# drscotthawley/flocoder

Measured on NVIDIA B200. Metric: samples/sec, 50-step RK4 latent sampling, higher is better.
Workload: dtype bf16

## Files before the change

### flocoder_b200/csrc/api.cu

```cuda
#include <cuda_fp16.h>
#include <math.h>
#include <stdarg.h>
#include <stdio.h>
#include <stdlib.h>
#include <string.h>

#include <algorithm>
#include <map>
#include <memory>
#include <string>
#include <vector>

#include "flo_internal.h"

namespace flo {

int conv_umma_smem_bytes(const ConvUmmaParams& p);

static thread_local std::string g_last_error;
void set_error(const char* fmt, ...) {
    char buf[1024];
    va_list ap;
    va_start(ap, fmt);
    vsnprintf(buf, sizeof(buf), fmt, ap);
// ... 1334 lines not shown
        }
    }
    for (size_t i = 0; i < h.bufs.size(); ++i) {
        const Buf& bf = h.bufs[i];
        snprintf(line, sizeof(line), "buf %3zu %-34s C=%d %dx%d %s bytes_ps=%zu live=[%d,%d] off_ps=%zu\n", i, bf.name.c_str(), bf.C, bf.H,
                 bf.W, bf.bf16 ? "bf16" : "f32 ", bf.bytes_ps, bf.def, bf.last, bf.off_ps);
        t += line;
    }
    if (h.spec.fused) {
        FusedBuilder fb(h, h.ftensors, h.fstages, 4);
        rc = fb.build();
        if (rc) return rc;
        snprintf(line, sizeof(line), "fused: %d stages, %d boundary tensors, %zu bytes/sample\n", (int)h.fstages.size(),
                 (int)h.ftensors.size(), h.farena_ps);
        t += line;
        for (size_t i = 0; i < h.fstages.size(); ++i) {
            const FStage& st = h.fstages[i];
            if (st.kind == 0) {
                const ChainParams& c = st.cp;
                snprintf(line, sizeof(line), "stage %2zu chain %-12s %dx%d nb=%d mt=%d strips=%d steps=%d loads=%d smem=%d (slots %d, ring %dx%d) tmem=%d nsplit=%d ctas=%d\n",
                         i, st.name.c_str(), c.H, c.W, c.nb, c.n_mtiles, c.strips, c.n_steps, c.n_loads, c.smem_bytes, c.ring_off,
                         c.n_ring, c.ring_slot_bytes, c.tmem_cols, c.nsplit, c.nsplit * ((B + c.nb - 1) / c.nb));
                t += line;
                for (int k = 0; k < c.n_steps; ++k) {
                    const ChainStep& cs = c.st[k];
                    snprintf(line, sizeof(line), "      step %d: conv=%d k=%d cin=%d+%d n=%d chunks=%dx%d res=%d(%dx%d) epi=%d C=%d G=%d film=%d resmode=%d out_slot=%d out_g=%d un=%d up=%d pn=%d final=%d a0=%d a1=%d\n",
                             k, cs.has_conv, cs.ksize, cs.a0_ncb * 8, cs.a1_ncb * 8, cs.n, cs.slices, cs.slices_per_chunk, cs.has_res,
                             cs.res_slices, cs.res_slices_per_chunk, cs.epi, cs.C, cs.groups, cs.film_off, cs.res_mode, cs.out_slot_off,
                             cs.out_g, cs.out_un_g, cs.out_up_g, cs.pn_g, cs.final, cs.a0_off, cs.a1_off);
                    t += line;
                }
            } else {
                const AttnFusedParams& a = st.ap;
                snprintf(line, sizeof(line), "stage %2zu attn  %-12s %dx%d C=%d nb=%d n=%d n_pad=%d mt=%d full=%d smem=%d plane=%d tmem=%d cols(k=%d v=%d ctx=%d q=%d out=%d proj=%d) ctas=%d\n",
                         i, st.name.c_str(), a.H, a.W, a.C, a.nb, a.n, a.n_pad, a.n_mtiles, a.full, a.smem_bytes, a.plane_bytes, a.tmem_cols,
                         a.col_k, a.col_v, a.col_ctx, a.col_q, a.col_out, a.col_proj, (B + a.nb - 1) / a.nb);
                t += line;
            }
        }
        for (size_t i = 0; i < h.ftensors.size(); ++i) {
            snprintf(line, sizeof(line), "ftensor %2zu %-24s C=%d %dx%d off_ps=%zu\n", i, h.ftensors[i].name.c_str(), h.ftensors[i].C,
                     h.ftensors[i].H, h.ftensors[i].W, h.ftensors[i].off_ps);
            t += line;
        }
    }
    if (out && cap > 0) snprintf(out, cap, "%s", t.c_str());
    return (int)t.size();
}

static void op_cost(const Handle& h, const Op& op, double& fl, double& by) {
    const Spec& s = h.spec;
    const double ob = s.bf16 ? 2.0 : 4.0;
    fl = 0; by = 0;
    const double hw = (double)op.H * op.W;
    switch (op.kind) {
        case OP_INIT:
            fl = 2.0 * hw * s.dim * s.channels;
            by = hw * (s.channels * 4.0 + s.dim * (ob + (s.bf16 ? 4.0 : 0.0)));
            break;
        case OP_CONV: {
            const double cin = (op.ncb0 + op.ncb1) * 8.0;
            fl = 2.0 * hw * op.cout * cin * op.ksize * op.ksize;
            by = hw * cin * ob + hw * op.cout * ((op.out_m >= 0 ? 4.0 : 0.0) + (op.out_o >= 0 ? ob : 0.0) + (op.res >= 0 ? 4.0 : 0.0));
        } break;
        case OP_GN:
            by = hw * op.C * (4.0 + (op.res >= 0 ? 4.0 : 0.0) + (op.out_m >= 0 ? 4.0 : 0.0) + (op.out_o >= 0 ? ob : 0.0) +
                              (op.out_un >= 0 ? ob : 0.0) + (op.out_up >= 0 ? 4.0 * ob : 0.0));
            fl = 10.0 * hw * op.C;
            break;
// ... 194 lines not shown
```

### flocoder_b200/csrc/flo_internal.h

```cpp
#pragma once
#include <cuda_runtime.h>
#include <cuda_bf16.h>
#include <cuda.h>
#include <stdint.h>
#include <string>
#include <vector>

#include "../../include/flocoder_b200.h"

namespace flo {

enum StageKind : int {
    ST_PLAIN = 0,
    ST_RK1 = 1,
    ST_RK2 = 2,
    ST_RK3 = 3,
    ST_RK4 = 4,
    ST_EULER = 5,
    ST_CFG_COND = 6
};
enum StageFlags : int {
    SF_CFG_COMBINE = 1,
    SF_CFG_2B = 2
};
// ... 204 lines not shown
    int ones_off;
    int fast;
    int max_c;
    int g_max, coef_n, cpar_n;
    int wide;
    int ring_off, ring_slot_bytes, n_ring, n_ring_deep;
    int stats_off, bar_off, smem_bytes, tmem_cols;
    int tab_off, tab_n;
    int wtab_off, n_chunks;
    int tabs_off;
    int nsplit;
    int xpart_off;
    int fmt;
    int film_dim;
    int cin0, dim, channels;
    int init_w_off, init_b_off, final_w_off, final_b_off;
    const uint16_t* wblob;
    const float* fblob;
    void* gt[CH_MAX_GT];
    Ctrl* ctrl;
    long long* dbg;
};

struct AttnFusedParams {
    int epi_warps;
    int B, H, W, C, nb, n, n_pad, n_mtiles;
    int full;
    int ktrans;
    int small;
    int fmt;
    unsigned wq_off, wk_off, wv_off, wo_off;
    int qkv_chunks, qkv_S, o_chunks, o_S;
    int bo_off, gamma_off, beta_off;
    int xh_off, p_off, v_off, ct_off, kmax_off, stats_off;
    int plane_bytes;
    int ring_off, ring_slot_bytes, n_ring, bar_off, smem_bytes, tmem_cols;
    int zero_off, zero_bytes;
    int col_k, col_v, col_ctx, col_q, col_out, col_proj;
    const uint16_t* wblob;
    const float* fblob;
    const void* x2;
    void* out; void* out_un; void* out_up;
    long long* dbg;
};

cudaError_t fused_configure();
int fused_max_active_clusters(int nsplit, int smem_bytes);
cudaError_t launch_chain(const ChainParams& p, const CUtensorMap* maps, int grid, cudaStream_t s);
cudaError_t launch_attn_fused(const AttnFusedParams& p, const CUtensorMap& xh_map, int grid, cudaStream_t s);


}
```

### flocoder_b200/csrc/fused_attn.cu

```cuda
#include "flo_internal.h"
#include "fused_common.cuh"

namespace flo {

struct RingA { int cc; };
__device__ __forceinline__ uint64_t desc64(uint32_t lo, uint32_t hi) {
    uint64_t d;
    asm("mov.b64 %0, {%1, %2};" : "=l"(d) : "r"(lo), "r"(hi));
    return d;
}
constexpr int ATTN_RING = 4;

__device__ __forceinline__ void attn_issue_chunk(const AttnFusedParams& p, uint32_t smem_base, uint32_t bar_full, uint32_t bar_empty,
                                                 int g, int qkv_bytes, int o_bytes) {
    const int qc = p.qkv_chunks;
    const uint16_t* w; int ci, bytes;
    if (g < qc) { w = p.wblob + p.wk_off; ci = g; bytes = qkv_bytes; }
    else if (g < 2 * qc) { w = p.wblob + p.wv_off; ci = g - qc; bytes = qkv_bytes; }
    else if (g < 3 * qc) { w = p.wblob + p.wq_off; ci = g - 2 * qc; bytes = qkv_bytes; }
    else { w = p.wblob + p.wo_off; ci = g - 3 * qc; bytes = o_bytes; }
    const int slot = g & (ATTN_RING - 1);
    if (g >= ATTN_RING) mbar_wait(bar_empty + 8 * slot, ((g / ATTN_RING) - 1) & 1);
    mbar_expect_tx(bar_full + 8 * slot, (uint32_t)bytes);
    bulk_load_1d(smem_base + p.ring_off + slot * p.ring_slot_bytes, reinterpret_cast<const uint8_t*>(w) + (size_t)ci * bytes,
// ... 86 lines not shown
}

template <int M>
__device__ __forceinline__ void colmax_halve(float (&v)[16], bool upper, int o) {
#pragma unroll
    for (int j = 0; j < M / 2; ++j) {
        const float send = upper ? v[j] : v[j + M / 2];
        const float keep = upper ? v[j + M / 2] : v[j];
        v[j] = fmaxf(keep, __shfl_xor_sync(0xffffffffu, send, o));
    }
}
template <int SEG>
__device__ __forceinline__ int colmax16(float (&v)[16], int lane) {
    int chan = 0;
    if (SEG == 32) {
        colmax_halve<16>(v, lane & 16, 16); chan += (lane & 16) ? 8 : 0;
        colmax_halve<8>(v, lane & 8, 8);    chan += (lane & 8) ? 4 : 0;
        colmax_halve<4>(v, lane & 4, 4);    chan += (lane & 4) ? 2 : 0;
        colmax_halve<2>(v, lane & 2, 2);    chan += (lane & 2) ? 1 : 0;
        v[0] = fmaxf(v[0], __shfl_xor_sync(0xffffffffu, v[0], 1));
    } else if (SEG == 16) {
        colmax_halve<16>(v, lane & 8, 8); chan += (lane & 8) ? 8 : 0;
        colmax_halve<8>(v, lane & 4, 4);  chan += (lane & 4) ? 4 : 0;
        colmax_halve<4>(v, lane & 2, 2);  chan += (lane & 2) ? 2 : 0;
        colmax_halve<2>(v, lane & 1, 1);  chan += (lane & 1) ? 1 : 0;
    } else {
        colmax_halve<16>(v, lane & 2, 2); chan += (lane & 2) ? 8 : 0;
        colmax_halve<8>(v, lane & 1, 1);  chan += (lane & 1) ? 4 : 0;
    }
    return chan;
}

template <int NT = 0, int FMTK = -1>
__global__ void __launch_bounds__(ATTN_MAX_THREADS) k_attn(const __grid_constant__ CUtensorMap tm_xh,
                                                        const __grid_constant__ AttnFusedParams p) {
    extern __shared__ __align__(128) uint8_t smem[];
    constexpr bool LEAN = NT > 0;
    const int fmt_k = FMTK >= 0 ? FMTK : p.fmt;
    const bool is_full = LEAN ? false : (p.full != 0);
    const bool is_kt = LEAN;
    const int warp = threadIdx.x >> 5, lane = threadIdx.x & 31, tid = threadIdx.x;
    const int EW = NT == 2 ? 16 : (NT == 1 ? 8 : p.epi_warps), n_epi = EW * 32, n_thr = (int)blockDim.x;
    const int n_mtiles_k = NT ? NT : p.n_mtiles;
    const bool n_ge32 = LEAN ? true : (p.n >= 32);
    const int w_prod = EW, w_mma = EW + 1;
    const uint32_t smem_base = smem_u32(smem);
    const uint32_t bar_full = smem_base + p.bar_off;
    const uint32_t bar_empty = bar_full + 8 * MAX_WSTAGES;
    const uint32_t bar_load = bar_empty + 8 * MAX_WSTAGES;
    const uint32_t bar_mma = bar_load + 8;
    const uint32_t bar_epi = bar_mma + 8;
    const uint32_t tmem_slot = bar_epi + 8;
    volatile uint32_t* tmem_slot_ptr = reinterpret_cast<volatile uint32_t*>(smem + p.bar_off + 16 * MAX_WSTAGES + 24);
    constexpr int NCH = 128;
    const int b0 = (int)blockIdx.x * p.nb;
    if (p.dbg && tid == 0 && blockIdx.x == 0) p.dbg[100] = global_ns();
    const int n = p.n, n_pad = p.n_pad, C = p.C;
    const uint32_t plane = (uint32_t)p.plane_bytes;
    const uint32_t xh_plane = (uint32_t)(p.nb * n) * 16u;
    const int lgn = 31 - __clz(n);
    const int mtS = (n + 127) >> 7;

    if (warp == w_prod && lane == 0) {
        for (int i = 0; i < p.n_ring; ++i) { mbar_init(bar_full + 8 * i, 1); mbar_init(bar_empty + 8 * i, 1); }
        mbar_init(bar_load, 1);
        mbar_init(bar_mma, 1);
        mbar_init(bar_epi, n_epi);
        asm volatile("fence.mbarrier_init.release.cluster;" ::: "memory");
    }
    if (warp == w_mma) tmem_alloc(tmem_slot, (uint32_t)p.tmem_cols);
    const bool all_live = !is_full && p.n_pad == p.n && ((p.nb * p.n) & 127) == 0 && b0 + p.nb <= p.B;
    if (!all_live)
        for (int i = tid * 16; i < p.zero_bytes; i += n_thr * 16)
            *reinterpret_cast<uint4*>(smem + p.zero_off + i) = make_uint4(0, 0, 0, 0);
    fence_proxy_async();
    tc_fence_before();
    __syncthreads();
    tc_fence_after();
    const uint32_t tmem_base = *tmem_slot_ptr;
    long long* dbg = (blockIdx.x == 0) ? p.dbg : nullptr;
    if (dbg && tid == 0) dbg[64] = clock64();
    if (dbg && tid == 0) dbg[101] = global_ns();
    const int qkv_bytes = p.qkv_S * 128 * 32, o_bytes = p.o_S * C * 32;

    if (warp == w_prod) {
        if (lane == 0) {
            const int total = 3 * p.qkv_chunks + p.o_chunks, pre = min(ATTN_RING, total);
            for (int g = 0; g < pre; ++g) attn_issue_chunk(p, smem_base, bar_full, bar_empty, g, qkv_bytes, o_bytes);
            griddep_wait();
            mbar_expect_tx(bar_load, (uint32_t)(C >> 3) * xh_plane);
            tma_load_5d(smem_base + p.xh_off, &tm_xh, bar_load, 0, 0, 0, b0, 0);
            for (int g = pre; g < total; ++g) attn_issue_chunk(p, smem_base, bar_full, bar_empty, g, qkv_bytes, o_bytes);
        }
    } else if (warp == w_mma) {
        {
            RingA rs{0};
            mbar_wait(bar_load, 0);
            tc_fence_after();
            if (dbg && lane == 0) dbg[0] = clock64();
            const bool tr = is_kt != 0;
            auto conv_T = [&](int col) {
                const uint32_t idesc = make_idesc16(128, p.nb * n, fmt_k, 0, 0);
                for (int ci = 0; ci < p.qkv_chunks; ++ci) {
                    const int slot = rs.cc & (ATTN_RING - 1);
                    mbar_wait(bar_full + 8 * slot, (rs.cc / ATTN_RING) & 1);
                    tc_fence_after();
                    if (elect_one()) {
                        for (int sl = 0; sl < p.qkv_S; ++sl) {
                            const uint32_t a_addr = smem_base + p.ring_off + (uint32_t)slot * (uint32_t)p.ring_slot_bytes + (uint32_t)sl * 4096u;
                            const uint32_t b_addr = smem_base + p.xh_off + (uint32_t)(ci * p.qkv_S + sl) * 2u * xh_plane;
                            umma_bf16(tmem_base + (uint32_t)col, make_smem_desc(a_addr, 2048u, 128u), make_smem_desc(b_addr, xh_plane, 128u), idesc,
                                      (ci * p.qkv_S + sl) > 0 ? 1u : 0u);
                        }
                        umma_commit(bar_empty + 8 * slot);
                    }
                    __syncwarp();
                    ++rs.cc;
                }
            };
            if (tr) {
// ... 2 lines not shown
            } else {
            attn_conv(p, smem_base, tmem_base, bar_full, bar_empty, rs, p.xh_off, xh_plane, NCH, 128, p.col_k, p.qkv_chunks, p.qkv_S);
            attn_conv(p, smem_base, tmem_base, bar_full, bar_empty, rs, p.xh_off, xh_plane, NCH, 128, p.col_v, p.qkv_chunks, p.qkv_S);
            }
            if (is_full) attn_conv(p, smem_base, tmem_base, bar_full, bar_empty, rs, p.xh_off, xh_plane, NCH, 128, p.col_q, p.qkv_chunks, p.qkv_S);
            if (dbg && lane == 0) dbg[1] = clock64();
            if (elect_one()) umma_commit(bar_mma);
            __syncwarp();
            int ph = 0;
            if (!is_full) {
                named_bar_sync(2, n_epi + 32); ++ph;
                tc_fence_after();
                if (dbg && lane == 0) dbg[8] = clock64();
                const uint32_t idesc_ctx = make_idesc16(128, NCH + 16, fmt_k, 1, 1);
                {
                    const int nb = p.nb, col_ctx = p.col_ctx;
                    const uint32_t p_off = p.p_off, v_off = p.v_off;
                    if (tr) {
                        const uint32_t idesc_t = make_idesc16(128, NCH + 16, fmt_k, 0, 0);
                        if (elect_one())
                            for (int s = 0; s < nb; ++s)
                                for (int ks = 0; ks < n / 16; ++ks) {
                                    const uint32_t pl = (uint32_t)(s * (n >> 3) + 2 * ks);
                                    umma_bf16(tmem_base + (uint32_t)(col_ctx + s * (NCH + 16)), make_smem_desc(smem_base + p_off + pl * 2048u, 2048u, 128u),
                                              make_smem_desc(smem_base + v_off + pl * 2304u, 2304u, 128u), idesc_t, ks > 0 ? 1u : 0u);
                                }
                    } else if (elect_one())
                        for (int s = 0; s < nb; ++s)
                            for (int ks = 0; ks < n_pad / 16; ++ks) {
                                const uint32_t roff = (uint32_t)(s * n_pad + ks * 16) * 16u;
                                umma_bf16(tmem_base + (uint32_t)(col_ctx + s * (NCH + 16)), make_smem_desc(smem_base + p_off + roff, 128u, plane),
                                          make_smem_desc(smem_base + v_off + roff, 128u, plane), idesc_ctx, ks > 0 ? 1u : 0u);
                            }
                    __syncwarp();
                }
                attn_conv(p, smem_base, tmem_base, bar_full, bar_empty, rs, p.xh_off, xh_plane, NCH, 128, p.col_q, p.qkv_chunks, p.qkv_S);
                if (dbg && lane == 0) dbg[9] = clock64();
                if (elect_one()) umma_commit(bar_mma);
                __syncwarp();
                named_bar_sync(2, n_epi + 32); ++ph;
                tc_fence_after();
                if (dbg && lane == 0) dbg[16] = clock64();
                const uint32_t idesc_out = make_idesc16(128, 32, fmt_k, 0, 0);
                {
                    const int nb = p.nb, col_out = p.col_out;
                    const uint32_t p_off = p.p_off, ct_off = p.ct_off;
                    if (elect_one()) {
                        for (int s = 0; s < nb; ++s)
                            for (int t = 0; t < mtS; ++t)
                                for (int h = 0; h < 4; ++h)
                                    for (int k = 0; k < 2; ++k) {
                                        const uint32_t a_addr = smem_base + p_off + (uint32_t)(4 * h + 2 * k) * plane +
                                                                (uint32_t)(s * n_pad + t * 128) * 16u;
                                        const uint32_t b_addr = smem_base + ct_off + (uint32_t)(s * 4 + h) * 2048u + (uint32_t)k * 1024u;
                                        umma_bf16(tmem_base + (uint32_t)(col_out + (s * mtS + t) * NCH + h * 32),
                                                  make_smem_desc(a_addr, plane, 128u), make_smem_desc(b_addr, 512u, 128u), idesc_out,
                                                  k > 0 ? 1u : 0u);
                                    }
                        umma_commit(bar_mma);
                    }
                    __syncwarp();
                }
            }
            named_bar_sync(2, n_epi + 32); ++ph;
            tc_fence_after();
            if (dbg && lane == 0) dbg[24] = clock64();
            attn_conv(p, smem_base, tmem_base, bar_full, bar_empty, rs, is_full ? p.p_off : p.v_off, plane, C, C, p.col_proj,
                      p.o_chunks, p.o_S);
            if (elect_one()) umma_commit(bar_mma);
            __syncwarp();
        }
    } else {
        const int quad = warp & 3, grp = warp >> 2;
        const int r = quad * 32 + lane;
        const int et = grp * 128 + r;
        const int half = EW == 16 ? (grp & 1) : 0;
        const int t0 = half, tstep = EW == 16 ? 2 : 1;
        const int cpart = EW == 16 ? (grp >> 1) : (EW == 8 ? grp : 0), ncp = EW >= 8 ? 2 : 1;
        const int ch_lo = cpart * (NCH / ncp), ch_hi = ch_lo + NCH / ncp;
        const uint32_t tlane = tmem_base + ((uint32_t)(quad * 32) << 16);
        auto esync = [&]() { named_bar_sync(1, n_epi); };
        float* kmax = reinterpret_cast<float*>(smem + p.kmax_off);
        float* kpart = kmax + p.nb * 128;
        float2* rowstat = reinterpret_cast<float2*>(smem + p.stats_off);
        float2* partial = rowstat + n_mtiles_k * 128;
        float2* stat = partial + 256;
        int ph = 0;
        float* par = reinterpret_cast<float*>(stat + 128);
        for (int c = et; c < C; c += n_epi) {
            par[c] = p.fblob[p.bo_off + c];
            par[128 + c] = is_full ? 1.0f : p.fblob[p.gamma_off + c];
            par[256 + c] = is_full ? 0.0f : p.fblob[p.beta_off + c];
        }
        esync();
        griddep_wait();
        mbar_wait(bar_load, 0);
        mbar_wait(bar_mma, ph & 1); ++ph;
        tc_fence_after();
        if (dbg && r == 0) dbg[2] = clock64();
        if (!is_full) {
          if (is_kt) {
            const int d = r;
            const int col0 = grp * 64, s = col0 >> lgn, gps = n >> 6;
            float mx = -INFINITY;
#pragma unroll
            for (int c = 0; c < 64; c += 32) {
                uint32_t ua[16], ub[16];
                tmem_ld16_issue(tlane + (uint32_t)(p.col_k + col0 + c), ua);
                tmem_ld16_issue(tlane + (uint32_t)(p.col_k + col0 + c + 16), ub);
                tmem_ld_wait();
                float m4[4] = {mx, -INFINITY, -INFINITY, -INFINITY};
#pragma unroll
                for (int j = 0; j < 16; ++j) { m4[j & 3] = fmaxf(m4[j & 3], __uint_as_float(ua[j])); m4[j & 3] = fmaxf(m4[j & 3], __uint_as_float(ub[j])); }
                mx = fmaxf(fmaxf(m4[0], m4[1]), fmaxf(m4[2], m4[3]));
            }
            kpart[grp * 128 + d] = mx;
            for (int pl = et; pl < (p.nb * n) >> 3; pl += n_epi) {
                const float ones[8] = {1.f, 1.f, 1.f, 1.f, 1.f, 1.f, 1.f, 1.f};
                *reinterpret_cast<uint4*>(smem + p.v_off + (uint32_t)pl * 2304u + 128u * 16u) = pack8(ones, fmt_k);
            }
            if (dbg && r == 0) dbg[3] = clock64();
            esync();
            for (int g = 0; g < gps; ++g) mx = fmaxf(mx, kpart[(s * gps + g) * 128 + d]);
#pragma unroll 2
            for (int c = 0; c < 64; c += 16) {
                uint32_t ku[16], vu[16];
// ... 84 lines not shown
                for (int c16 = ch_lo; c16 < ch_hi; c16 += 16) {
                    uint32_t ku[16], vu[16];
                    tmem_ld16_issue(tlane + (uint32_t)(p.col_k + t * NCH + c16), ku);
                    tmem_ld16_issue(tlane + (uint32_t)(p.col_v + t * NCH + c16), vu);
                    tmem_ld_wait();
                    if (!valid) continue;
                    float kv[16], vv[16];
#pragma unroll
                    for (int j = 0; j < 16; ++j) { kv[j] = __uint_as_float(ku[j]); vv[j] = __uint_as_float(vu[j]); }
                    const float4* km4 = reinterpret_cast<const float4*>(kmax + s * 128 + c16);
#pragma unroll
                    for (int k4 = 0; k4 < 4; ++k4) {
                        const float4 m4 = km4[k4];
                        kv[4 * k4] = fast_exp(kv[4 * k4] - m4.x); kv[4 * k4 + 1] = fast_exp(kv[4 * k4 + 1] - m4.y);
                        kv[4 * k4 + 2] = fast_exp(kv[4 * k4 + 2] - m4.z); kv[4 * k4 + 3] = fast_exp(kv[4 * k4 + 3] - m4.w);
                    }
                    uint8_t* pd = smem + p.p_off + (uint32_t)(c16 >> 3) * plane + row_off;
                    uint8_t* vd = smem + p.v_off + (uint32_t)(c16 >> 3) * plane + row_off;
                    *reinterpret_cast<uint4*>(pd) = pack8(kv, fmt_k);
                    *reinterpret_cast<uint4*>(pd + plane) = pack8(kv + 8, fmt_k);
                    *reinterpret_cast<uint4*>(vd) = pack8(vv, fmt_k);
                    *reinterpret_cast<uint4*>(vd + plane) = pack8(vv + 8, fmt_k);
                }
                if (valid && cpart == 0) {
                    const float ones[8] = {1.f, 1.f, 1.f, 1.f, 1.f, 1.f, 1.f, 1.f};
                    *reinterpret_cast<uint4*>(smem + p.v_off + (uint32_t)(NCH >> 3) * plane + row_off) = pack8(ones, fmt_k);
                }
            }
            if (dbg && r == 0) dbg[4] = clock64();
            fence_proxy_async();
            tc_fence_before();
            named_bar_arrive(2, n_epi + 32);
          }
            mbar_wait(bar_mma, ph & 1); ++ph;
            tc_fence_after();
            if (dbg && r == 0) dbg[10] = clock64();
            {
                const int h = quad, d = lane;
                for (int s = t0; s < p.nb; s += tstep) {
                    uint32_t u0[16], u1[16], us[16];
                    tmem_ld16_issue(tlane + (uint32_t)(p.col_ctx + s * (NCH + 16) + h * 32), u0);
                    tmem_ld16_issue(tlane + (uint32_t)(p.col_ctx + s * (NCH + 16) + h * 32 + 16), u1);
                    tmem_ld16_issue(tlane + (uint32_t)(p.col_ctx + s * (NCH + 16) + NCH), us);
                    tmem_ld_wait();
                    const int e_lo = cpart * (32 / ncp), e_hi = e_lo + 32 / ncp;
                    float c0[16], c1[16];
#pragma unroll
                    for (int j = 0; j < 16; ++j) { c0[j] = __uint_as_float(u0[j]); c1[j] = __uint_as_float(u1[j]); }
                    const float inv = 0.17677669529663687f * fast_rcp(__uint_as_float(us[0]));
                    uint8_t* base = smem + p.ct_off + (uint32_t)(s * 4 + h) * 2048u + (uint32_t)(d >> 3) * 512u + (uint32_t)(d & 7) * 2u;
#pragma unroll
                    for (int e = 0; e < 32; ++e) {
                        if (e < e_lo || e >= e_hi) continue;
                        const float val = (e < 16 ? c0[e] : c1[e - 16]) * inv;
                        const uint32_t u = pack2(val, 0.f, fmt_k);
                        *reinterpret_cast<uint16_t*>(base + (uint32_t)(e >> 3) * 128u + (uint32_t)(e & 7) * 16u) = (uint16_t)(u & 0xFFFFu);
                    }
                }
            }
            for (int t = t0; t < n_mtiles_k; t += tstep) {
                const int rd = t * 128 + r, s = rd >> lgn, px = rd & (n - 1);
                const bool valid = s < p.nb && b0 + s < p.B;
                const uint32_t row_off = (uint32_t)(s * n_pad + px) * 16u;
                for (int h2 = cpart * (4 / ncp); h2 < (cpart + 1) * (4 / ncp); h2 += 2) {
                    uint32_t qu[2][32];
#pragma unroll
                    for (int k = 0; k < 2; ++k) {
                        tmem_ld16_issue(tlane + (uint32_t)(p.col_q + t * NCH + (h2 + k) * 32), *reinterpret_cast<uint32_t(*)[16]>(&qu[k][0]));
                        tmem_ld16_issue(tlane + (uint32_t)(p.col_q + t * NCH + (h2 + k) * 32 + 16), *reinterpret_cast<uint32_t(*)[16]>(&qu[k][16]));
                    }
                    tmem_ld_wait();
                    if (!valid) continue;
#pragma unroll
                    for (int k = 0; k < 2; ++k) {
                        float q[32];
#pragma unroll
                        for (int j = 0; j < 32; ++j) q[j] = __uint_as_float(qu[k][j]);
                        float m4[4] = {q[0], q[1], q[2], q[3]};
#pragma unroll
                        for (int j = 4; j < 32; ++j) m4[j & 3] = fmaxf(m4[j & 3], q[j]);
                        const float m = fmaxf(fmaxf(m4[0], m4[1]), fmaxf(m4[2], m4[3]));
                        float s4[4] = {0.f, 0.f, 0.f, 0.f};
#pragma unroll
                        for (int j = 0; j < 32; ++j) { q[j] = fast_exp(q[j] - m); s4[j & 3] += q[j]; }
                        const float inv = fast_rcp((s4[0] + s4[1]) + (s4[2] + s4[3]));
#pragma unroll
                        for (int j = 0; j < 32; ++j) q[j] *= inv;
                        uint8_t* qd = smem + p.p_off + (uint32_t)(4 * (h2 + k)) * plane + row_off;
#pragma unroll
                        for (int cb = 0; cb < 4; ++cb) *reinterpret_cast<uint4*>(qd + (uint32_t)cb * plane) = pack8(q + cb * 8, fmt_k);
                    }
                }
            }
            if (dbg && r == 0) dbg[11] = clock64();
            fence_proxy_async();
            tc_fence_before();
            named_bar_arrive(2, n_epi + 32);
            mbar_wait(bar_mma, ph & 1); ++ph;
            tc_fence_after();
            if (dbg && r == 0) dbg[18] = clock64();
            for (int s = 0; s < p.nb; ++s)
                for (int t = (mtS > 1 ? t0 : 0); t < mtS; t += (mtS > 1 ? tstep : 1)) {
                    const int px = t * 128 + r;
                    const bool valid = px < n && b0 + s < p.B;
                    const uint32_t row_off = (uint32_t)(s * n + px) * 16u;
                    for (int c32 = ch_lo; c32 < ch_hi; c32 += 32) {
                        uint32_t ua[16], ub[16];
                        tmem_ld16_issue(tlane + (uint32_t)(p.col_out + (s * mtS + t) * NCH + c32), ua);
                        tmem_ld16_issue(tlane + (uint32_t)(p.col_out + (s * mtS + t) * NCH + c32 + 16), ub);
                        tmem_ld_wait();
                        if (!valid) continue;
                        float v[32];
#pragma unroll
                        for (int j = 0; j < 16; ++j) { v[j] = __uint_as_float(ua[j]); v[16 + j] = __uint_as_float(ub[j]); }
                        uint8_t* od = smem + p.v_off + (uint32_t)(c32 >> 3) * plane + row_off;
#pragma unroll
                        for (int k8 = 0; k8 < 4; ++k8) *reinterpret_cast<uint4*>(od + (uint32_t)k8 * plane) = pack8(v + 8 * k8, fmt_k);
                    }
                }
            fence_proxy_async();
            tc_fence_before();
            named_bar_arrive(2, n_epi + 32);
        } else {
            constexpr uint32_t KP = 272u;
            constexpr int QP = 132;
            uint8_t* kbuf = smem + p.v_off;
            uint8_t* vbuf = kbuf + 32 * KP;
            float* qbuf = reinterpret_cast<float*>(vbuf + 32 * KP);
            if (warp == 0) {
                for (int c16 = 0; c16 < 128; c16 += 16) {
                    uint32_t ku[16], vu[16], qu[16];
                    tmem_ld16_issue(tlane + (uint32_t)(p.col_k + c16), ku);
                    tmem_ld16_issue(tlane + (uint32_t)(p.col_v + c16), vu);
                    tmem_ld16_issue(tlane + (uint32_t)(p.col_q + c16), qu);
                    tmem_ld_wait();
                    float kv[16], vv[16], qv[16];
#pragma unroll
                    for (int j = 0; j < 16; ++j) { kv[j] = __uint_as_float(ku[j]); vv[j] = __uint_as_float(vu[j]); qv[j] = __uint_as_float(qu[j]); }
                    const uint32_t kvrow = (uint32_t)((lane & (n - 1)) * p.nb + (lane >> lgn));
                    uint8_t* kd = kbuf + kvrow * KP + (uint32_t)c16 * 2u;
                    uint8_t* vd = vbuf + kvrow * KP + (uint32_t)c16 * 2u;
                    *reinterpret_cast<uint4*>(kd) = pack8(kv, fmt_k);
                    *reinterpret_cast<uint4*>(kd + 16) = pack8(kv + 8, fmt_k);
                    *reinterpret_cast<uint4*>(vd) = pack8(vv, fmt_k);
                    *reinterpret_cast<uint4*>(vd + 16) = pack8(vv + 8, fmt_k);
                    float4* qd = reinterpret_cast<float4*>(qbuf + lane * QP + c16);
#pragma unroll
                    for (int k4 = 0; k4 < 4; ++k4) qd[k4] = make_float4(qv[4 * k4], qv[4 * k4 + 1], qv[4 * k4 + 2], qv[4 * k4 + 3]);
                }
            }
            esync();
            {
// ... 49 lines not shown
                    }
                }
                if (!valid) {
#pragma unroll
                    for (int e = 0; e < 32; ++e) o[e] = 0.f;
                }
#pragma unroll
                for (int cb = 0; cb < 4; ++cb)
                    *reinterpret_cast<uint4*>(smem + p.p_off + (uint32_t)(4 * h + cb) * plane + (uint32_t)row * 16u) = pack8(o + cb * 8, fmt_k);
            }
            fence_proxy_async();
            tc_fence_before();
            named_bar_arrive(2, n_epi + 32);
        }
        if (dbg && r == 0) dbg[19] = clock64();
        uint4 pre_xa = make_uint4(0, 0, 0, 0), pre_xb = pre_xa;
        if (!is_full && t0 < n_mtiles_k && cpart == 0) {
            const int rd = t0 * 128 + r, s = rd >> lgn, px = rd & (n - 1);
            if (s < p.nb && b0 + s < p.B) {
                const uint4* xsrc = reinterpret_cast<const uint4*>(p.x2);
                pre_xa = xsrc[(size_t)(0 * p.B + b0 + s) * n + px];
                pre_xb = xsrc[(size_t)(1 * p.B + b0 + s) * n + px];
            }
        }
        mbar_wait(bar_mma, ph & 1); ++ph;
        tc_fence_after();
        if (dbg && r == 0) dbg[26] = clock64();
        griddep_launch();
        const float* bias = par;
        if (!is_full) {
            for (int t = t0; t < n_mtiles_k && cpart == 0; t += tstep) {
                const int rd = t * 128 + r, s = rd >> lgn;
                const bool valid = s < p.nb && b0 + s < p.B;
                float sx = 0.f, sq = 0.f;
                float sx2 = 0.f, sq2 = 0.f;
                for (int c16 = 0; c16 < C; c16 += 32) {
                    uint32_t ua[16], ub[16];
                    const bool two = c16 + 16 < C;
                    tmem_ld16_issue(tlane + (uint32_t)(p.col_proj + t * C + c16), ua);
                    if (two) tmem_ld16_issue(tlane + (uint32_t)(p.col_proj + t * C + c16 + 16), ub);
                    tmem_ld_wait();
#pragma unroll
                    for (int j = 0; j < 16; ++j) { const float x = __uint_as_float(ua[j]) + bias[c16 + j]; sx += x; sq += x * x; }
                    if (two) {
#pragma unroll
                        for (int j = 0; j < 16; ++j) { const float x = __uint_as_float(ub[j]) + bias[c16 + 16 + j]; sx2 += x; sq2 += x * x; }
                    }
                }
                sx += sx2; sq += sq2;
                if (n_ge32) {
                    if (!valid) { sx = 0.f; sq = 0.f; }
                    for (int o = 16; o > 0; o >>= 1) { sx += __shfl_xor_sync(0xffffffffu, sx, o); sq += __shfl_xor_sync(0xffffffffu, sq, o); }
                    if (lane == 0) partial[rd >> 5] = make_float2(sx, sq);
                } else {
                    rowstat[rd] = valid ? make_float2(sx, sq) : make_float2(0.f, 0.f);
                }
            }
            int parts = 1;
            while (parts * 2 * p.nb <= 128 && parts < 16) parts *= 2;
            if (dbg && et == 0) dbg[27] = clock64();
            esync();
            if (dbg && et == 0) dbg[28] = clock64();
            if (n_ge32) {
                if (et < p.nb) {
                    const int bps = n >> 5;
                    float tx = 0.f, tq = 0.f;
#pragma unroll
                    for (int k = 0; k < 8; ++k)
                        if (k < bps) { const float2 a = partial[et * bps + k]; tx += a.x; tq += a.y; }
                    const float icnt = fast_rcp((float)(C * n));
                    const float mean = tx * icnt;
                    stat[et] = make_float2(mean, rsqrtf(fmaxf(tq * icnt - mean * mean, 0.f) + 1e-5f));
                }
// ... 27 lines not shown
            float* ybuf = reinterpret_cast<float*>(smem + p.v_off);
            if (warp == 0) {
                for (int c16 = 0; c16 < C; c16 += 16) {
                    float v[16];
                    tmem_ld16(tlane + (uint32_t)(p.col_proj + c16), v);
                    float4* yd = reinterpret_cast<float4*>(ybuf + lane * QP + c16);
#pragma unroll
                    for (int k4 = 0; k4 < 4; ++k4) yd[k4] = make_float4(v[4 * k4], v[4 * k4 + 1], v[4 * k4 + 2], v[4 * k4 + 3]);
                }
            }
            esync();
            const int row = lane, s = row >> lgn, px = row & (n - 1), b = b0 + s;
            if (b < p.B) {
                const uint4* xsrc = reinterpret_cast<const uint4*>(p.x2);
                for (int c16 = warp * 16; c16 < C; c16 += 64) {
                    const uint4 xa = xsrc[(size_t)((c16 >> 3) * p.B + b) * n + px];
                    const uint4 xb = xsrc[(size_t)(((c16 >> 3) + 1) * p.B + b) * n + px];
                    float v[16], x2[16];
                    const float4* ys = reinterpret_cast<const float4*>(ybuf + row * QP + c16);
#pragma unroll
                    for (int k4 = 0; k4 < 4; ++k4) { const float4 t4 = ys[k4]; v[4 * k4] = t4.x; v[4 * k4 + 1] = t4.y; v[4 * k4 + 2] = t4.z; v[4 * k4 + 3] = t4.w; }
                    unpack8(xa, x2, fmt_k);
                    unpack8(xb, x2 + 8, fmt_k);
#pragma unroll
                    for (int j = 0; j < 16; ++j) v[j] = v[j] + bias[c16 + j] + x2[j];
                    attn_write_out(p, b, px, c16, v, fmt_k);
                }
            }
        } else {
            for (int t = t0; t < n_mtiles_k && cpart == 0; t += tstep) {
                const int rd = t * 128 + r, s = rd >> lgn, px = rd & (n - 1);
                const bool valid = s < p.nb && b0 + s < p.B;
                const int b = b0 + s;
                float2 ms = make_float2(0.f, 1.f);
                if (s < p.nb) ms = stat[s];
                if (dbg && et == 0) dbg[30] = clock64();
                const uint4* xsrc = reinterpret_cast<const uint4*>(p.x2);
                uint4 xa = pre_xa, xb = pre_xb;
                if (valid && t != t0) { xa = xsrc[(size_t)(0 * p.B + b) * n + px]; xb = xsrc[(size_t)(1 * p.B + b) * n + px]; }
                for (int c16 = 0; c16 < C; c16 += 16) {
                    uint4 na = make_uint4(0, 0, 0, 0), nb4 = na;
                    if (valid && c16 + 16 < C) {
                        na = xsrc[(size_t)(((c16 >> 3) + 2) * p.B + b) * n + px];
                        nb4 = xsrc[(size_t)(((c16 >> 3) + 3) * p.B + b) * n + px];
                    }
                    float v[16], x2[16];
                    tmem_ld16(tlane + (uint32_t)(p.col_proj + t * C + c16), v);
                    if (valid) {
                        unpack8(xa, x2, fmt_k);
                        unpack8(xb, x2 + 8, fmt_k);
#pragma unroll
                        for (int j = 0; j < 16; ++j) {
                            const float y = (v[j] + bias[c16 + j] - ms.x) * ms.y * gamma[c16 + j] + beta[c16 + j];
                            v[j] = y + x2[j];
                        }
                    }
                    attn_write_out_w(p, b, px, c16, v, valid, fmt_k);
                    xa = na; xb = nb4;
                }
            }
        }
        if (dbg && et == 0) dbg[29] = clock64();
    }
    tc_fence_before();
    __syncthreads();
    if (dbg && tid == 0) dbg[65] = clock64();
    if (p.dbg && tid == 0) { if (blockIdx.x == 0) p.dbg[102] = global_ns(); atomicMax(reinterpret_cast<unsigned long long*>(p.dbg + 103), (unsigned long long)global_ns()); }
    if (warp == w_mma) tmem_dealloc(tmem_base, (uint32_t)p.tmem_cols);
}

constexpr uint32_t SM_KP = 528u;
constexpr int SMALL_EW = 16;
constexpr int SMALL_THREADS = (SMALL_EW + 2) * 32;
template <int SEG, bool IS_MAX>
__device__ __forceinline__ int segred16(float (&v)[16], int lane) {
    int chan = 0;
    auto halve = [&](int m, bool upper, int o) {
#pragma unroll
        for (int j = 0; j < 8; ++j) {
            if (j < m / 2) {
// ... 502 lines not shown
```

### flocoder_b200/csrc/fused_plan.inc

```

struct FusedBuilder {
    Handle& h;
    const Spec& s;
    std::vector<FTensor>& T;
    std::vector<FStage>& S;
    bool debug;
    int qcap;
    FusedBuilder(Handle& hh, std::vector<FTensor>& t, std::vector<FStage>& st, int qcap_)
        : h(hh), s(hh.spec), T(t), S(st), debug((hh.spec.flags & FLO_FLAG_NO_BUFFER_REUSE) != 0), qcap(qcap_) {}

    int tensor(const std::string& name, int C, int H, int W) {
        for (size_t i = 0; i < T.size(); ++i)
            if (T[i].name == name) return (int)i;
        FTensor t; t.name = name; t.C = C; t.H = H; t.W = W;
        t.bytes_ps = ((size_t)C * H * W * 2 + 255) & ~(size_t)255; t.off_ps = 0;
        T.push_back(t);
        return (int)T.size() - 1;
    }
    const Op& op(const std::string& name, int kind) {
        for (auto& o : h.ops)
            if (o.name == name && o.kind == kind) return o;
        set_error("internal: no op '%s'", name.c_str());
        throw 1;
    }
// ... 336 lines not shown
            a.qkv_S = std::max(1, std::min(C / 16, 8192 / (128 * 32)));
            while ((C / 16) % a.qkv_S) --a.qkv_S;
            a.qkv_chunks = (C / 16) / a.qkv_S;
            const Op& o = full ? op(p, OP_CONV) : op(p + ".fn.fn.to_out.0", OP_CONV);
            a.wo_off = (unsigned)o.w_umma; a.bo_off = (int)o.bias;
            if (!full) { const Op& g = op(p, OP_GN); a.gamma_off = (int)g.gamma; a.beta_off = (int)g.beta; }
            a.o_S = std::max(1, std::min(8, 8192 / (C * 32)));
            while (8 % a.o_S) --a.o_S;
            a.o_chunks = 8 / a.o_S;
            a.plane_bytes = 2048;
            int off = 0;
            a.xh_off = off; off += std::max((C / 8) * 2048, 16 * 2048);
            a.p_off = off; off += 128 * 528;
            a.v_off = off; off += 128 * 528;
            a.kmax_off = off; off += 16 * 2 * (32 / n) * 16 * 4;
            a.stats_off = off; off += 2 * 64 * 8 + 3 * 128 * 4;
            a.zero_off = 0; a.zero_bytes = 0;
            a.n_ring = 4;
            a.ring_slot_bytes = std::max(a.qkv_S * 128 * 32, a.o_S * C * 32);
            a.ring_off = (off + 127) & ~127; off = a.ring_off + a.n_ring * a.ring_slot_bytes;
            a.bar_off = off; off += 16 * MAX_WSTAGES + 64;
            a.smem_bytes = off;
            if (off > 227 * 1024) { set_error("attention %s needs %d bytes of shared memory", p.c_str(), off); return FLO_ERR_UNSUPPORTED; }
            a.tmem_cols = 512; a.col_k = 0; a.col_v = 128; a.col_q = 256; a.col_proj = 384;
            S.push_back(st);
            return FLO_OK;
        }
        if (full) {
            if (n > 16 || 32 % n) { set_error("mid attention supports H*W in {1,2,4,8,16}, got %d", n); return FLO_ERR_UNSUPPORTED; }
            a.nb = 32 / n; a.n_pad = n;
        } else {
            if (n != 256 && (n > 128 || 128 % n)) { set_error("linear attention: unsupported H*W=%d", n); return FLO_ERR_UNSUPPORTED; }
            a.n_pad = std::max(n, 16);
            a.nb = n >= 128 ? 1 : 2;
        }
        st.nb = a.nb;
        a.n_mtiles = (a.nb * n + 127) / 128;
        const int nch = 128;
        const Op& qkv = op(p + ".fn.fn.to_qkv", OP_CONV);
        const unsigned per_tile = (unsigned)(C / 16) * 128u * 16u;
        a.wq_off = (unsigned)qkv.w_umma; a.wk_off = a.wq_off + per_tile; a.wv_off = a.wq_off + 2 * per_tile;
        chunking(C / 16, 128, a.qkv_chunks, a.qkv_S);
        if (full) {
            const Op& o = op(p, OP_CONV);
            a.wo_off = (unsigned)o.w_umma; a.bo_off = (int)o.bias; a.gamma_off = 0; a.beta_off = 0;
        } else {
            const Op& o = op(p + ".fn.fn.to_out.0", OP_CONV);
            const Op& g = op(p, OP_GN);
            a.wo_off = (unsigned)o.w_umma; a.bo_off = (int)o.bias; a.gamma_off = (int)g.gamma; a.beta_off = (int)g.beta;
        }
        chunking(nch / 16, C, a.o_chunks, a.o_S);
        const int npx = std::max(a.n_mtiles * 128, a.nb * a.n_pad);
        a.plane_bytes = npx * 16;
        int off = 0;
        a.xh_off = off; off += ((C / 8) * a.nb * n * 16 + 127) & ~127;
        a.zero_off = off;
        a.p_off = off; off += (nch / 8) * a.plane_bytes;
        a.v_off = off; off += (nch / 8 + 2) * a.plane_bytes;
        a.ct_off = off; off += full ? 0 : a.nb * 4 * 2048;
        a.zero_bytes = off - a.zero_off;
        off += (a.nb * n % 128) ? 2048 : 0;
        a.kmax_off = off; off += full ? 0 : (a.nb + a.n_mtiles * 4) * 128 * 4;
        a.epi_warps = full ? 4 : (a.n_mtiles == 2 ? 16 : 8);
        a.stats_off = off; off += (a.n_mtiles * 128 + 256 + 128) * 8 + 3 * 128 * 4;
        a.n_ring = 4;
        a.ring_slot_bytes = std::max(a.qkv_S * 128 * 32, a.o_S * C * 32);
        a.ring_off = (off + 127) & ~127; off = a.ring_off + a.n_ring * a.ring_slot_bytes;
        a.bar_off = off; off += 16 * MAX_WSTAGES + 64;
        a.smem_bytes = off;
        if (off > 227 * 1024) { set_error("attention %s needs %d bytes of shared memory", p.c_str(), off); return FLO_ERR_UNSUPPORTED; }
        a.ktrans = (!full && n >= 64 && a.nb * n <= 256 && (a.nb * n) / (a.epi_warps / 4) == 64 &&
                    !getenv("FLO_ATTN_NO_KTRANS")) ? 1 : 0;
        a.tmem_cols = 512;
        if (full) { a.col_k = 0; a.col_v = 128; a.col_q = 256; a.col_proj = 384; }
        else {
            a.col_k = 0; a.col_v = a.n_mtiles * nch; a.col_ctx = 0;
            a.col_q = std::max(a.n_mtiles * nch, a.nb * (nch + 16));
            a.col_out = 0; a.col_proj = 256;
            if (a.col_q + a.n_mtiles * nch > a.tmem_cols || a.col_proj + a.n_mtiles * C > a.tmem_cols) { set_error("attention %s: TMEM plan does not fit", p.c_str()); return FLO_ERR_UNSUPPORTED; }
        }
        if (a.tmem_cols > 256) a.smem_bytes = std::max(a.smem_bytes, 117 * 1024);
        S.push_back(st);
        return FLO_OK;
    }

    int build() {
        try {
            const int n = s.n_levels;
            std::vector<int> Hs(n), Ws(n);
            for (int l = 0; l < n; ++l) { Hs[l] = s.H >> l; Ws[l] = s.W >> l; }
            const int t_r = tensor("init_conv", s.dim, s.H, s.W);
            std::vector<int> skipA(n), skipB(n);
            int t_un = -1;
            for (int l = 0; l < n; ++l) {
                const int C = s.dims[l], H = Hs[l], W = Ws[l];
                const std::string p = "downs." + std::to_string(l);
                const bool last = l == n - 1;
                begin_chain("S_down" + std::to_string(l), H, W, l == 0 ? s.dim : C);
                int sx;
                if (l == 0) {
                    mark_epi_slots();
                    ChainStep& st = new_step();
                    st.epi = CE_INIT; st.C = s.dim;
                    sx = slot(s.dim);
                    st.out_slot_off = sx; st.out_g = gt(t_r);
                } else {
                    const int su = load(t_un);
                    sx = conv_bias("downs." + std::to_string(l - 1) + ".3", su, s.dims[l - 1] * 4, C,
                                   debug ? tensor("downs." + std::to_string(l - 1) + ".3", C, H, W) : -1);
                    release(su, s.dims[l - 1] * 4);
                }
                skipA[l] = tensor(p + ".0", C, H, W);
// ... 174 lines not shown
```

Before: 4192.

## Fold attention context into output projection weights before the final MMA

Linear attention previously computed out = q·ctx with one MMA, wrote the result back to shared memory, then ran a second MMA for the output projection. The epilogue now folds the normalized context matrix into the to_out weights (M = ctx·Wo) with packed FMA on CUDA cores, using weights staged in shared memory. A single MMA of q against M then produces the projection directly, removing one MMA pass, one TMEM round trip and one barrier phase. The change also stops streaming the to_out weights through the ring for non-full attention, sets nb=1 for n<32, and tightens launch bounds for NT==1. In exchange it adds CUDA-core FMA work in the epilogue and needs extra shared memory.

```diff
diff --git a/flocoder_b200/csrc/api.cu b/flocoder_b200/csrc/api.cu
--- a/flocoder_b200/csrc/api.cu
+++ b/flocoder_b200/csrc/api.cu
@@ -1390,9 +1390,9 @@
                 }
             } else {
                 const AttnFusedParams& a = st.ap;
-                snprintf(line, sizeof(line), "stage %2zu attn  %-12s %dx%d C=%d nb=%d n=%d n_pad=%d mt=%d full=%d smem=%d plane=%d tmem=%d cols(k=%d v=%d ctx=%d q=%d out=%d proj=%d) ctas=%d\n",
+                snprintf(line, sizeof(line), "stage %2zu attn  %-12s %dx%d C=%d nb=%d n=%d n_pad=%d mt=%d full=%d smem=%d plane=%d tmem=%d cols(k=%d v=%d ctx=%d q=%d proj=%d) ctas=%d\n",
                          i, st.name.c_str(), a.H, a.W, a.C, a.nb, a.n, a.n_pad, a.n_mtiles, a.full, a.smem_bytes, a.plane_bytes, a.tmem_cols,
-                         a.col_k, a.col_v, a.col_ctx, a.col_q, a.col_out, a.col_proj, (B + a.nb - 1) / a.nb);
+                         a.col_k, a.col_v, a.col_ctx, a.col_q, a.col_proj, (B + a.nb - 1) / a.nb);
                 t += line;
             }
         }
diff --git a/flocoder_b200/csrc/flo_internal.h b/flocoder_b200/csrc/flo_internal.h
--- a/flocoder_b200/csrc/flo_internal.h
+++ b/flocoder_b200/csrc/flo_internal.h
@@ -260,11 +260,11 @@
     unsigned wq_off, wk_off, wv_off, wo_off;
     int qkv_chunks, qkv_S, o_chunks, o_S;
     int bo_off, gamma_off, beta_off;
-    int xh_off, p_off, v_off, ct_off, kmax_off, stats_off;
+    int xh_off, p_off, v_off, m_off, wf_off, kmax_off, stats_off;
     int plane_bytes;
     int ring_off, ring_slot_bytes, n_ring, bar_off, smem_bytes, tmem_cols;
     int zero_off, zero_bytes;
-    int col_k, col_v, col_ctx, col_q, col_out, col_proj;
+    int col_k, col_v, col_ctx, col_q, col_proj;
     const uint16_t* wblob;
     const float* fblob;
     const void* x2;
diff --git a/flocoder_b200/csrc/fused_attn.cu b/flocoder_b200/csrc/fused_attn.cu
--- a/flocoder_b200/csrc/fused_attn.cu
+++ b/flocoder_b200/csrc/fused_attn.cu
@@ -142,7 +142,7 @@
 }
 
 template <int NT = 0, int FMTK = -1>
-__global__ void __launch_bounds__(ATTN_MAX_THREADS) k_attn(const __grid_constant__ CUtensorMap tm_xh,
+__global__ void __launch_bounds__(NT == 1 ? 320 : ATTN_MAX_THREADS) k_attn(const __grid_constant__ CUtensorMap tm_xh,
                                                         const __grid_constant__ AttnFusedParams p) {
     extern __shared__ __align__(128) uint8_t smem[];
     constexpr bool LEAN = NT > 0;
@@ -161,6 +161,7 @@
     const uint32_t bar_mma = bar_load + 8;
     const uint32_t bar_epi = bar_mma + 8;
     const uint32_t tmem_slot = bar_epi + 8;
+    const uint32_t bar_ctx = bar_epi + 16;
     volatile uint32_t* tmem_slot_ptr = reinterpret_cast<volatile uint32_t*>(smem + p.bar_off + 16 * MAX_WSTAGES + 24);
     constexpr int NCH = 128;
     const int b0 = (int)blockIdx.x * p.nb;
@@ -169,13 +170,13 @@
     const uint32_t plane = (uint32_t)p.plane_bytes;
     const uint32_t xh_plane = (uint32_t)(p.nb * n) * 16u;
     const int lgn = 31 - __clz(n);
-    const int mtS = (n + 127) >> 7;
 
     if (warp == w_prod && lane == 0) {
         for (int i = 0; i < p.n_ring; ++i) { mbar_init(bar_full + 8 * i, 1); mbar_init(bar_empty + 8 * i, 1); }
         mbar_init(bar_load, 1);
         mbar_init(bar_mma, 1);
         mbar_init(bar_epi, n_epi);
+        mbar_init(bar_ctx, 1);
         asm volatile("fence.mbarrier_init.release.cluster;" ::: "memory");
     }
     if (warp == w_mma) tmem_alloc(tmem_slot, (uint32_t)p.tmem_cols);
@@ -195,7 +196,7 @@
 
     if (warp == w_prod) {
         if (lane == 0) {
-            const int total = 3 * p.qkv_chunks + p.o_chunks, pre = min(ATTN_RING, total);
+            const int total = 3 * p.qkv_chunks + (is_full ? p.o_chunks : 0), pre = min(ATTN_RING, total);
             for (int g = 0; g < pre; ++g) attn_issue_chunk(p, smem_base, bar_full, bar_empty, g, qkv_bytes, o_bytes);
             griddep_wait();
             mbar_expect_tx(bar_load, (uint32_t)(C >> 3) * xh_plane);
@@ -264,41 +265,29 @@
                                 umma_bf16(tmem_base + (uint32_t)(col_ctx + s * (NCH + 16)), make_smem_desc(smem_base + p_off + roff, 128u, plane),
                                           make_smem_desc(smem_base + v_off + roff, 128u, plane), idesc_ctx, ks > 0 ? 1u : 0u);
                             }
+                    if (elect_one()) umma_commit(bar_ctx);
                     __syncwarp();
                 }
                 attn_conv(p, smem_base, tmem_base, bar_full, bar_empty, rs, p.xh_off, xh_plane, NCH, 128, p.col_q, p.qkv_chunks, p.qkv_S);
                 if (dbg && lane == 0) dbg[9] = clock64();
                 if (elect_one()) umma_commit(bar_mma);
                 __syncwarp();
-                named_bar_sync(2, n_epi + 32); ++ph;
-                tc_fence_after();
-                if (dbg && lane == 0) dbg[16] = clock64();
-                const uint32_t idesc_out = make_idesc16(128, 32, fmt_k, 0, 0);
-                {
-                    const int nb = p.nb, col_out = p.col_out;
-                    const uint32_t p_off = p.p_off, ct_off = p.ct_off;
-                    if (elect_one()) {
-                        for (int s = 0; s < nb; ++s)
-                            for (int t = 0; t < mtS; ++t)
-                                for (int h = 0; h < 4; ++h)
-                                    for (int k = 0; k < 2; ++k) {
-                                        const uint32_t a_addr = smem_base + p_off + (uint32_t)(4 * h + 2 * k) * plane +
-                                                                (uint32_t)(s * n_pad + t * 128) * 16u;
-                                        const uint32_t b_addr = smem_base + ct_off + (uint32_t)(s * 4 + h) * 2048u + (uint32_t)k * 1024u;
-                                        umma_bf16(tmem_base + (uint32_t)(col_out + (s * mtS + t) * NCH + h * 32),
-                                                  make_smem_desc(a_addr, plane, 128u), make_smem_desc(b_addr, 512u, 128u), idesc_out,
-                                                  k > 0 ? 1u : 0u);
-                                    }
-                        umma_commit(bar_mma);
-                    }
-                    __syncwarp();
-                }
             }
             named_bar_sync(2, n_epi + 32); ++ph;
             tc_fence_after();
             if (dbg && lane == 0) dbg[24] = clock64();
-            attn_conv(p, smem_base, tmem_base, bar_full, bar_empty, rs, is_full ? p.p_off : p.v_off, plane, C, C, p.col_proj,
-                      p.o_chunks, p.o_S);
+            if (is_full) {
+                attn_conv(p, smem_base, tmem_base, bar_full, bar_empty, rs, p.p_off, plane, C, C, p.col_proj, p.o_chunks, p.o_S);
+            } else if (elect_one()) {
+                const int nbc = p.nb * C;
+                const uint32_t idesc_o = make_idesc16(128, nbc, fmt_k, 0, 0);
+                for (int t = 0; t < n_mtiles_k; ++t)
+                    for (int sl = 0; sl < NCH / 16; ++sl)
+                        umma_bf16(tmem_base + (uint32_t)(p.col_proj + t * nbc),
+                                  make_smem_desc(smem_base + p.p_off + (uint32_t)sl * 2u * plane + (uint32_t)t * 2048u, plane, 128u),
+                                  make_smem_desc(smem_base + p.m_off + (uint32_t)(sl * nbc) * 32u, (uint32_t)nbc * 16u, 128u), idesc_o,
+                                  sl > 0 ? 1u : 0u);
+            }
             if (elect_one()) umma_commit(bar_mma);
             __syncwarp();
         }
@@ -324,6 +313,12 @@
             par[128 + c] = is_full ? 1.0f : p.fblob[p.gamma_off + c];
             par[256 + c] = is_full ? 0.0f : p.fblob[p.beta_off + c];
         }
+        const uint4* w16 = reinterpret_cast<const uint4*>(smem + p.wf_off);
+        if (!is_full) {
+            const uint4* wsrc = reinterpret_cast<const uint4*>(p.wblob + p.wo_off);
+            for (int i = et; i < C * (NCH / 8); i += n_epi)
+                reinterpret_cast<uint4*>(smem + p.wf_off)[i] = wsrc[(i & 15) * C + (i >> 4)];
+        }
         esync();
         griddep_wait();
         mbar_wait(bar_load, 0);
@@ -474,36 +469,70 @@
             tc_fence_before();
             named_bar_arrive(2, n_epi + 32);
           }
-            mbar_wait(bar_mma, ph & 1); ++ph;
+            mbar_wait(bar_ctx, 0);
             tc_fence_after();
             if (dbg && r == 0) dbg[10] = clock64();
             {
                 const int h = quad, d = lane;
-                for (int s = t0; s < p.nb; s += tstep) {
-                    uint32_t u0[16], u1[16], us[16];
-                    tmem_ld16_issue(tlane + (uint32_t)(p.col_ctx + s * (NCH + 16) + h * 32), u0);
-                    tmem_ld16_issue(tlane + (uint32_t)(p.col_ctx + s * (NCH + 16) + h * 32 + 16), u1);
-                    tmem_ld16_issue(tlane + (uint32_t)(p.col_ctx + s * (NCH + 16) + NCH), us);
-                    tmem_ld_wait();
-                    const int e_lo = cpart * (32 / ncp), e_hi = e_lo + 32 / ncp;
-                    float c0[16], c1[16];
-#pragma unroll
-                    for (int j = 0; j < 16; ++j) { c0[j] = __uint_as_float(u0[j]); c1[j] = __uint_as_float(u1[j]); }
-                    const float inv = 0.17677669529663687f * fast_rcp(__uint_as_float(us[0]));
-                    uint8_t* base = smem + p.ct_off + (uint32_t)(s * 4 + h) * 2048u + (uint32_t)(d >> 3) * 512u + (uint32_t)(d & 7) * 2u;
-#pragma unroll
-                    for (int e = 0; e < 32; ++e) {
-                        if (e < e_lo || e >= e_hi) continue;
-                        const float val = (e < 16 ? c0[e] : c1[e - 16]) * inv;
-                        const uint32_t u = pack2(val, 0.f, fmt_k);
-                        *reinterpret_cast<uint16_t*>(base + (uint32_t)(e >> 3) * 128u + (uint32_t)(e & 7) * 16u) = (uint16_t)(u & 0xFFFFu);
-                    }
-                }
-            }
+                const int cper = C / (EW >> 2), c_lo = grp * cper;
+                const int nbc = p.nb * C, k = h * 32 + d;
+                uint8_t* mrow = smem + p.m_off + (uint32_t)(k >> 4) * (uint32_t)(nbc * 32) + (uint32_t)((k >> 3) & 1) * (uint32_t)(nbc * 16) +
+                                (uint32_t)(k & 7) * 2u;
+                auto fold = [&](auto ns_tag, int s0) {
+                    constexpr int NS = decltype(ns_tag)::value;
+                    float2 cx[NS][16];
+                    float inv[NS];
+#pragma unroll
+                    for (int s = 0; s < NS; ++s) {
+                        uint32_t u0[16], u1[16], us[16];
+                        const int cc = p.col_ctx + (s0 + s) * (NCH + 16);
+                        tmem_ld16_issue(tlane + (uint32_t)(cc + h * 32), u0);
+                        tmem_ld16_issue(tlane + (uint32_t)(cc + h * 32 + 16), u1);
+                        tmem_ld16_issue(tlane + (uint32_t)(cc + NCH), us);
+                        tmem_ld_wait();
+#pragma unroll
+                        for (int j = 0; j < 8; ++j) {
+                            cx[s][j] = make_float2(__uint_as_float(u0[2 * j]), __uint_as_float(u0[2 * j + 1]));
+                            cx[s][8 + j] = make_float2(__uint_as_float(u1[2 * j]), __uint_as_float(u1[2 * j + 1]));
+                        }
+                        inv[s] = 0.17677669529663687f * fast_rcp(__uint_as_float(us[0]));
+                    }
+#pragma unroll 1
+                    for (int c = c_lo; c < c_lo + cper; ++c) {
+                        const uint4* w8 = w16 + c * (NCH / 8) + h * 4;
+                        float2 a0[NS], a1[NS];
+#pragma unroll
+                        for (int s = 0; s < NS; ++s) { a0[s] = make_float2(0.f, 0.f); a1[s] = a0[s]; }
+#pragma unroll
+                        for (int j = 0; j < 4; ++j) {
+                            const uint4 u = w8[j];
+                            const float2 wa = unpack2(u.x, fmt_k), wb = unpack2(u.y, fmt_k), wc = unpack2(u.z, fmt_k), wd = unpack2(u.w, fmt_k);
+#pragma unroll
+                            for (int s = 0; s < NS; ++s) {
+                                a0[s] = __ffma2_rn(wa, cx[s][4 * j], a0[s]);
+                                a1[s] = __ffma2_rn(wb, cx[s][4 * j + 1], a1[s]);
+                                a0[s] = __ffma2_rn(wc, cx[s][4 * j + 2], a0[s]);
+                                a1[s] = __ffma2_rn(wd, cx[s][4 * j + 3], a1[s]);
+                            }
+                        }
+#pragma unroll
+                        for (int s = 0; s < NS; ++s) {
+                            const int nr = (s0 + s) * C + c;
+                            const uint32_t u = pack2(((a0[s].x + a0[s].y) + (a1[s].x + a1[s].y)) * inv[s], 0.f, fmt_k);
+                            *reinterpret_cast<uint16_t*>(mrow + (uint32_t)(nr >> 3) * 128u + (uint32_t)(nr & 7) * 16u) = (uint16_t)(u & 0xFFFFu);
+                        }
+                    }
+                };
+                if (NT == 1 && p.nb == 2) fold(std::integral_constant<int, 2>{}, 0);
+                else
+                    for (int s0 = 0; s0 < p.nb; ++s0) fold(std::integral_constant<int, 1>{}, s0);
+            }
+            mbar_wait(bar_mma, ph & 1); ++ph;
+            tc_fence_after();
             for (int t = t0; t < n_mtiles_k; t += tstep) {
-                const int rd = t * 128 + r, s = rd >> lgn, px = rd & (n - 1);
+                const int rd = t * 128 + r, s = rd >> lgn;
                 const bool valid = s < p.nb && b0 + s < p.B;
-                const uint32_t row_off = (uint32_t)(s * n_pad + px) * 16u;
+                const uint32_t row_off = (uint32_t)rd * 16u;
                 for (int h2 = cpart * (4 / ncp); h2 < (cpart + 1) * (4 / ncp); h2 += 2) {
                     uint32_t qu[2][32];
 #pragma unroll
@@ -535,31 +564,6 @@
                 }
             }
             if (dbg && r == 0) dbg[11] = clock64();
-            fence_proxy_async();
-            tc_fence_before();
-            named_bar_arrive(2, n_epi + 32);
-            mbar_wait(bar_mma, ph & 1); ++ph;
-            tc_fence_after();
-            if (dbg && r == 0) dbg[18] = clock64();
-            for (int s = 0; s < p.nb; ++s)
-                for (int t = (mtS > 1 ? t0 : 0); t < mtS; t += (mtS > 1 ? tstep : 1)) {
-                    const int px = t * 128 + r;
-                    const bool valid = px < n && b0 + s < p.B;
-                    const uint32_t row_off = (uint32_t)(s * n + px) * 16u;
-                    for (int c32 = ch_lo; c32 < ch_hi; c32 += 32) {
-                        uint32_t ua[16], ub[16];
-                        tmem_ld16_issue(tlane + (uint32_t)(p.col_out + (s * mtS + t) * NCH + c32), ua);
-                        tmem_ld16_issue(tlane + (uint32_t)(p.col_out + (s * mtS + t) * NCH + c32 + 16), ub);
-                        tmem_ld_wait();
-                        if (!valid) continue;
-                        float v[32];
-#pragma unroll
-                        for (int j = 0; j < 16; ++j) { v[j] = __uint_as_float(ua[j]); v[16 + j] = __uint_as_float(ub[j]); }
-                        uint8_t* od = smem + p.v_off + (uint32_t)(c32 >> 3) * plane + row_off;
-#pragma unroll
-                        for (int k8 = 0; k8 < 4; ++k8) *reinterpret_cast<uint4*>(od + (uint32_t)k8 * plane) = pack8(v + 8 * k8, fmt_k);
-                    }
-                }
             fence_proxy_async();
             tc_fence_before();
             named_bar_arrive(2, n_epi + 32);
@@ -675,13 +679,14 @@
             for (int t = t0; t < n_mtiles_k && cpart == 0; t += tstep) {
                 const int rd = t * 128 + r, s = rd >> lgn;
                 const bool valid = s < p.nb && b0 + s < p.B;
+                const int pcol = p.col_proj + t * p.nb * C + min(s, p.nb - 1) * C;
                 float sx = 0.f, sq = 0.f;
                 float sx2 = 0.f, sq2 = 0.f;
                 for (int c16 = 0; c16 < C; c16 += 32) {
                     uint32_t ua[16], ub[16];
                     const bool two = c16 + 16 < C;
-                    tmem_ld16_issue(tlane + (uint32_t)(p.col_proj + t * C + c16), ua);
-                    if (two) tmem_ld16_issue(tlane + (uint32_t)(p.col_proj + t * C + c16 + 16), ub);
+                    tmem_ld16_issue(tlane + (uint32_t)(pcol + c16), ua);
+                    if (two) tmem_ld16_issue(tlane + (uint32_t)(pcol + c16 + 16), ub);
                     tmem_ld_wait();
 #pragma unroll
                     for (int j = 0; j < 16; ++j) { const float x = __uint_as_float(ua[j]) + bias[c16 + j]; sx += x; sq += x * x; }
@@ -775,6 +780,7 @@
                 const int rd = t * 128 + r, s = rd >> lgn, px = rd & (n - 1);
                 const bool valid = s < p.nb && b0 + s < p.B;
                 const int b = b0 + s;
+                const int pcol = p.col_proj + t * p.nb * C + min(s, p.nb - 1) * C;
                 float2 ms = make_float2(0.f, 1.f);
                 if (s < p.nb) ms = stat[s];
                 if (dbg && et == 0) dbg[30] = clock64();
@@ -788,7 +794,7 @@
                         nb4 = xsrc[(size_t)(((c16 >> 3) + 3) * p.B + b) * n + px];
                     }
                     float v[16], x2[16];
-                    tmem_ld16(tlane + (uint32_t)(p.col_proj + t * C + c16), v);
+                    tmem_ld16(tlane + (uint32_t)(pcol + c16), v);
                     if (valid) {
                         unpack8(xa, x2, fmt_k);
                         unpack8(xb, x2 + 8, fmt_k);
diff --git a/flocoder_b200/csrc/fused_plan.inc b/flocoder_b200/csrc/fused_plan.inc
--- a/flocoder_b200/csrc/fused_plan.inc
+++ b/flocoder_b200/csrc/fused_plan.inc
@@ -392,7 +392,7 @@
         } else {
             if (n != 256 && (n > 128 || 128 % n)) { set_error("linear attention: unsupported H*W=%d", n); return FLO_ERR_UNSUPPORTED; }
             a.n_pad = std::max(n, 16);
-            a.nb = n >= 128 ? 1 : 2;
+            a.nb = (n >= 128 || n < 32) ? 1 : 2;
         }
         st.nb = a.nb;
         a.n_mtiles = (a.nb * n + 127) / 128;
@@ -417,9 +417,10 @@
         a.zero_off = off;
         a.p_off = off; off += (nch / 8) * a.plane_bytes;
         a.v_off = off; off += (nch / 8 + 2) * a.plane_bytes;
-        a.ct_off = off; off += full ? 0 : a.nb * 4 * 2048;
         a.zero_bytes = off - a.zero_off;
         off += (a.nb * n % 128) ? 2048 : 0;
+        a.m_off = off; off += full ? 0 : a.nb * C * nch * 2;
+        a.wf_off = off; off += full ? 0 : C * nch * 2;
         a.kmax_off = off; off += full ? 0 : (a.nb + a.n_mtiles * 4) * 128 * 4;
         a.epi_warps = full ? 4 : (a.n_mtiles == 2 ? 16 : 8);
         a.stats_off = off; off += (a.n_mtiles * 128 + 256 + 128) * 8 + 3 * 128 * 4;
@@ -436,8 +437,10 @@
         else {
             a.col_k = 0; a.col_v = a.n_mtiles * nch; a.col_ctx = 0;
             a.col_q = std::max(a.n_mtiles * nch, a.nb * (nch + 16));
-            a.col_out = 0; a.col_proj = 256;
-            if (a.col_q + a.n_mtiles * nch > a.tmem_cols || a.col_proj + a.n_mtiles * C > a.tmem_cols) { set_error("attention %s: TMEM plan does not fit", p.c_str()); return FLO_ERR_UNSUPPORTED; }
+            a.col_proj = 256;
+            if (a.col_q + a.n_mtiles * nch > a.tmem_cols || a.col_proj + a.n_mtiles * a.nb * C > a.tmem_cols || a.nb * C > 256) {
+                set_error("attention %s: TMEM plan does not fit", p.c_str()); return FLO_ERR_UNSUPPORTED;
+            }
         }
         if (a.tmem_cols > 256) a.smem_bytes = std::max(a.smem_bytes, 117 * 1024);
         S.push_back(st);
```

Measured after the change: 4219 (median of 6 runs). About the same (+0.7%).
